# 0xEigenLabs/eigen-zkvm

Measured on AMD Instinct MI355X. Metric: Goldilocks NTT GElems/s + BN254 G1 MSM Mpts/s; starky prove ms at 2^24 rows, higher is better.
Workload: dtype u64 (Goldilocks, canonical)

## Files before the change

### eigen-zkvm_amd/csrc/ntt.hip

```cpp
#include "zk_internal.h"
#include "ntt_reg.hip.h"
#include <map>
#include <mutex>
#include <type_traits>
#include <vector>

namespace zk {

namespace {

constexpr int NTT_TILE = 4096;
constexpr int TW_LO_BITS = 12;
constexpr int TW_LO = 1 << TW_LO_BITS;

struct PassParams {
    const u64* in;
    u64* out;
    const u64* w256;
    const u64* tw_lo;
    const u64* tw_hi;
    const u64* tw_mid;
    u64 pre_scale;
    u32 dshift;
    const u64* sc_lo;
    const u64* sc_hi;
    u64 sc_cinv;
    u64 out_scale;
    u64 inner;
    u64 valid_in;
    u64 s_np;
    u32 np;
    u32 log_s;
    u32 has_tw;
};

__device__ __forceinline__ u64 tab2(const u64* __restrict__ lo, const u64* __restrict__ hi, u64 e) {
    return gl::mul_tw_nc(hi[e >> TW_LO_BITS], lo[e & (TW_LO - 1)]);
}

template <int LOGA, int LOGB, bool KMODE, bool INV>
__global__ __launch_bounds__(NTT_TILE / 16) void ntt_pass_kernel(const PassParams P) {
    constexpr int LOGR = LOGA + LOGB, R = 1 << LOGR, RA = 1 << LOGA, RB = 1 << LOGB;
    constexpr int C = NTT_TILE / R;
    constexpr int GA = 16 / RA, GB = 16 / RB;
    constexpr int TG = R / 16;
    constexpr int PAD = KMODE ? 512 / R : 0;
    constexpr int ROW = RB * C + PAD;
    static_assert(LOGR >= 4 && LOGR <= 8 && LOGA <= 4 && LOGB <= 4, "tile shape");
    __shared__ u64 lds[RA * ROW];
    __shared__ u64 sfac[RB * C];

    const int t = threadIdx.x;
    const u64 u0 = (u64)blockIdx.x * C;

    auto split = [&](u64 u, u64& p, u64& rem) {
        const u64 uc = u < P.inner ? u : 0;
        if (P.np == 1) { p = uc >> P.log_s; rem = uc & (((u64)1 << P.log_s) - 1); }
        else if ((P.inner >> 32) == 0) { const u32 p32 = (u32)uc / (u32)P.s_np; p = p32; rem = (u32)uc - p32 * (u32)P.s_np; }
        else
        { p = uc / P.s_np; rem = uc - p * P.s_np; }
    };
    auto row_of = [&](u64 rem) { return P.np == 1 ? rem : (P.inner >> 32) == 0 ? (u64)((u32)rem / P.np) : rem / P.np; };
    const bool small = ((P.inner * R) >> 29) == 0;
    int cB, tb;
    if (KMODE) { tb = t % TG; cB = t / TG; } else { cB = t % C; tb = t / C; }

    const bool split_f = (P.has_tw && !P.tw_mid) || P.sc_lo;
    u64 fa_hi[GB], fa_lo[GB], fs_hi[GA], fs_lo[GA], fa[GB];
#pragma unroll
    for (int g = 0; g < GB; ++g) fa_hi[g] = fa_lo[g] = fa[g] = 1;
#pragma unroll
    for (int m = 0; m < GA; ++m) fs_hi[m] = fs_lo[m] = 1;
    auto issue_factor_loads = [&]() {
        const u64* __restrict__ lo = P.sc_lo ? P.sc_lo : P.tw_lo;
        const u64* __restrict__ hi = P.sc_lo ? P.sc_hi : P.tw_hi;
        u64 p, rem;
        split(u0 + cB, p, rem);
        const u32 rq = P.sc_lo ? (u32)row_of(rem) : 0;
#pragma unroll
        for (int g = 0; g < GB; ++g) {
            const u32 ka = tb + g * TG;
            const u32 e = P.sc_lo ? (ka << P.log_s) + rq : ((u32)p * ka) << P.log_s;
            fa_hi[g] = hi[e >> TW_LO_BITS]; fa_lo[g] = lo[e & (TW_LO - 1)];
        }
#pragma unroll
        for (int m = 0; m < GA; ++m) {
            const int i = t + m * (NTT_TILE / 16);
            const u32 kb = i / C;
            split(u0 + i % C, p, rem);
            const u32 e = P.sc_lo ? (RA * kb) << P.log_s : ((u32)p * (RA * kb)) << P.log_s;
            fs_hi[m] = hi[e >> TW_LO_BITS]; fs_lo[m] = lo[e & (TW_LO - 1)];
        }
    };

    {
        const int c = t % C, ta = t / C;
        const u64 u = u0 + c;
        const bool live = u < P.inner;
        u64 x[GA][RA];
        const bool full = u0 + C <= P.inner && (u64)(R - 1) * P.inner + u0 + C <= P.valid_in;
        const u64* __restrict__ base = P.in + (u64)(ta * GA) * P.inner + (live ? u : 0);
        if (full) {
#pragma unroll
            for (int g = 0; g < GA; ++g)
#pragma unroll
                for (int ja = 0; ja < RA; ++ja) x[g][ja] = base[(u64)(ja * RB + g) * P.inner];
        } else {
#pragma unroll
            for (int g = 0; g < GA; ++g)
#pragma unroll
                for (int ja = 0; ja < RA; ++ja) {
                    const u64 off = (u64)(ja * RB + g) * P.inner;
                    const bool ok = live && (u64)(ta * GA) * P.inner + off + u < P.valid_in;
                    const u64 v = *(ok ? base + off : P.in);
                    x[g][ja] = ok ? v : 0;
                }
        }
        if (split_f) issue_factor_loads();
#pragma unroll
        for (int g = 0; g < GA; ++g) ntt_reg<LOGA, INV>(x[g]);
        if (LOGR <= 6 && C >= 64 && LOGB > 0 && P.pre_scale == 1) {
            static_for<0, TG>([&](auto TA) {
                constexpr int ta_c = decltype(TA)::value;
                if (ta == ta_c) {
                    static_for<0, GA>([&](auto GI) {
                        constexpr int g = decltype(GI)::value, jb = ta_c * GA + g;
                        static_for<0, RA>([&](auto KA) {
                            constexpr int ka = decltype(KA)::value;
                            constexpr int e0 = (39 * (64 / (R > 64 ? 64 : R)) * jb * ka) % 192, e = INV ? (192 - e0) % 192 : e0;
                            u64 v = x[g][bitrev_c(ka, LOGA)];
                            if constexpr (e >= 96) v = gl::neg(gl::mul_pow2<e - 96>(v));
                            else v = gl::mul_pow2<e>(v);
                            lds[ka * ROW + jb * C + c] = v;
                        });
                    });
                }
            });
        } else
        {
#pragma unroll
            for (int g = 0; g < GA; ++g) {
                const int jb = ta * GA + g;
#pragma unroll
                for (int ka = 0; ka < RA; ++ka) {
                    u64 v = x[g][bitrev_c(ka, LOGA)];
                    if (LOGB > 0 && ka > 0) v = gl::mul_tw(v, P.w256[(jb * ka) << (8 - LOGR)]);
                    else if (P.pre_scale != 1) v = gl::mul_tw(v, P.pre_scale);
                    lds[ka * ROW + jb * C + c] = v;
                }
            }
        }
    }
    if (split_f) {
#pragma unroll
        for (int m = 0; m < GA; ++m) {
            u64 sv = gl::mul_tw_nc(fs_hi[m], fs_lo[m]);
            if (P.sc_lo) sv = gl::mul_tw_nc(sv, P.sc_cinv);
            sfac[t + m * (NTT_TILE / 16)] = sv;
        }
#pragma unroll
        for (int g = 0; g < GB; ++g) fa[g] = gl::mul_tw_nc(fa_hi[g], fa_lo[g]);
    }
    __syncthreads();
    {
        const int c = cB;
        const u64 u = u0 + c;
        u64 y[GB][RB];
#pragma unroll
        for (int g = 0; g < GB; ++g) {
            const int ka = tb + g * TG;
#pragma unroll
            for (int jb = 0; jb < RB; ++jb) y[g][jb] = lds[ka * ROW + jb * C + c];
        }
        u64 p, rem;
        split(u, p, rem);
        u64 tw[GB][RB];
        if (P.tw_mid) {
            const u32 sh = P.log_s - P.dshift, istep = (((u32)p * RA) << sh) * 8;
#pragma unroll
            for (int g = 0; g < GB; ++g) {
                const u32 ka = tb + g * TG, i0 = (((u32)p * ka) << sh) * 8;
#pragma unroll
                for (int kb = 0; kb < RB; ++kb) tw[g][kb] = *(const u64*)((const char*)P.tw_mid + (u32)(i0 + kb * istep));
            }
        }
#pragma unroll
        for (int g = 0; g < GB; ++g) ntt_reg<LOGB, INV>(y[g]);
        if (u >= P.inner) return;

        auto finish = [&](auto small_c) {
            constexpr bool SMALL = decltype(small_c)::value;
            u64* __restrict__ outp = P.out + p * R * P.s_np + rem;
            const u64 kstride = P.s_np;
            const u32 b0 = ((u32)p * R * (u32)P.s_np + (u32)rem) * 8, bstep = RA * (u32)P.s_np * 8;
            auto put = [&](int g, int kb, u64 v) {
                const u32 ka = tb + g * TG;
                if constexpr (SMALL) *(u64*)((char*)P.out + (u32)(b0 + ka * (u32)P.s_np * 8 + kb * bstep)) = v;
                else outp[(u64)(RA * kb + ka) * kstride] = v;
            };
            if (P.tw_mid) {
#pragma unroll
                for (int g = 0; g < GB; ++g)
#pragma unroll
                    for (int kb = 0; kb < RB; ++kb) put(g, kb, gl::mul_tw(y[g][bitrev_c(kb, LOGB)], tw[g][kb]));
            } else if (split_f) {
#pragma unroll
                for (int g = 0; g < GB; ++g)
#pragma unroll
                    for (int kb = 0; kb < RB; ++kb) {
                        const u64 f = kb == 0 ? fa[g] : gl::mul_tw_nc(fa[g], sfac[kb * C + c]);
                        put(g, kb, gl::mul_tw(y[g][bitrev_c(kb, LOGB)], f));
                    }
            } else if (P.out_scale != 1) {
#pragma unroll
                for (int g = 0; g < GB; ++g)
#pragma unroll
                    for (int kb = 0; kb < RB; ++kb) put(g, kb, gl::mul_tw(y[g][bitrev_c(kb, LOGB)], P.out_scale));
            } else {
#pragma unroll
                for (int g = 0; g < GB; ++g)
#pragma unroll
                    for (int kb = 0; kb < RB; ++kb) put(g, kb, y[g][bitrev_c(kb, LOGB)]);
            }
        };
        if (small) finish(std::true_type{});
        else finish(std::false_type{});
    }
}

__global__ void ntt_small_kernel(const u64* in, u64* out, u32 np, u32 n_in, u32 n, u64 w, u64 g, u64 cst) {
    const u32 tid = blockIdx.x * blockDim.x + threadIdx.x;
    if (tid >= n * np) return;
    const u32 k = tid / np, c = tid % np;
    const u64 wk = gl::pow(w, k);
    u64 acc = 0, cur = 1;
    for (u32 i = 0; i < n_in; ++i) { acc = gl::add(acc, gl::mul(in[(u64)i * np + c], cur)); cur = gl::mul(cur, wk); }
    out[(u64)k * np + c] = gl::mul(acc, gl::mul(cst, gl::pow(g, k)));
}

struct Tables { DevConst w256, w256s, lo, hi, mid; u32 dshift = 0; };
struct ScaleTables { DevConst lo, hi; };

std::mutex g_mu;
auto& g_tables = *new std::map<std::pair<int, std::pair<u32, int>>, Tables>;
auto& g_scales = *new std::map<std::pair<int, std::pair<u32, u64>>, ScaleTables>;

void two_level(u64 base, u64 cst, u32 nbits, std::vector<u64>& lo, std::vector<u64>& hi) {
    lo.resize(TW_LO);
    u64 c = cst;
    for (int i = 0; i < TW_LO; ++i) { lo[i] = c; c = gl::hmul(c, base); }
    size_t nh = nbits > (u32)TW_LO_BITS ? (size_t)1 << (nbits - TW_LO_BITS) : 1;
    hi.resize(nh);
    u64 step = gl::hpow(base, TW_LO);
    c = 1;
    for (size_t i = 0; i < nh; ++i) { hi[i] = c; c = gl::hmul(c, step); }
}

const Tables& get_tables(u32 nbits, bool inverse) {
    int dev; ZK_HIP(hipGetDevice(&dev));
    std::lock_guard<std::mutex> lk(g_mu);
    auto key = std::make_pair(dev, std::make_pair(nbits, (int)inverse));
    auto it = g_tables.find(key);
    if (it != g_tables.end()) return it->second;
    u64 w = gl::hroot(nbits), w8 = gl::hroot(8);
    if (inverse) { w = gl::hinv(w); w8 = gl::hinv(w8); }
    std::vector<u64> t256(256), lo, hi;
    u64 c = 1;
    for (int i = 0; i < 256; ++i) { t256[i] = c; c = gl::hmul(c, w8); }
    two_level(w, 1, nbits, lo, hi);
    Tables T; T.w256 = DevConst(t256); T.lo = DevConst(lo); T.hi = DevConst(hi);
    if (inverse) {
        const u64 ninv = gl::hinv((1ull << nbits) % GL_P);
        std::vector<u64> t256s(256);
        for (int i = 0; i < 256; ++i) t256s[i] = gl::hmul(t256[i], ninv);
        T.w256s = DevConst(t256s);
    }
    {
        T.dshift = nbits > 16 ? nbits - 16 : 0;
        const size_t nm = (size_t)1 << (nbits - T.dshift);
        std::vector<u64> mid(nm);
        const u64 step = gl::hpow(w, 1ull << T.dshift);
        c = 1;
        for (size_t i = 0; i < nm; ++i) { mid[i] = c; c = gl::hmul(c, step); }
        T.mid = DevConst(mid);
    }
    return g_tables.emplace(key, std::move(T)).first->second;
}

const ScaleTables& get_scale(u32 nbits, u64 g, u64 cst) {
    int dev; ZK_HIP(hipGetDevice(&dev));
    std::lock_guard<std::mutex> lk(g_mu);
    auto key = std::make_pair(dev, std::make_pair(nbits, g));
    auto it = g_scales.find(key);
    if (it != g_scales.end()) return it->second;
    std::vector<u64> lo, hi;
    two_level(g, cst, nbits, lo, hi);
    ScaleTables S; S.lo = DevConst(lo); S.hi = DevConst(hi);
    return g_scales.emplace(key, std::move(S)).first->second;
}

template <int LOGA, int LOGB>
void launch_pass(const PassParams& P, bool kmode, bool inverse, hipStream_t st) {
    constexpr int C = NTT_TILE >> (LOGA + LOGB);
    const u64 blocks = (P.inner + C - 1) / C;
    ZK_REQUIRE(blocks < (1ull << 31), "ntt: grid too large");
    const dim3 g((u32)blocks), b(NTT_TILE / 16);
    const int variant = (kmode ? 2 : 0) | (inverse ? 1 : 0);
#define ZK_PASS(K, I) hipLaunchKernelGGL((ntt_pass_kernel<LOGA, LOGB, K, I>), g, b, 0, st, P)
    switch (variant) {
        case 0: ZK_PASS(false, false); break; case 1: ZK_PASS(false, true); break;
        case 2: ZK_PASS(true, false); break;  default: ZK_PASS(true, true); break;
    }
#undef ZK_PASS
    ZK_HIP(hipGetLastError());
}

void launch_pass_logr(int logr, const PassParams& P, bool kmode, bool inverse, hipStream_t st) {
    switch (logr) {
        case 4: launch_pass<2, 2>(P, kmode, inverse, st); break;
        case 5: launch_pass<3, 2>(P, kmode, inverse, st); break;
        case 6: launch_pass<3, 3>(P, kmode, inverse, st); break;
        case 7: launch_pass<4, 3>(P, kmode, inverse, st); break;
        case 8: launch_pass<4, 4>(P, kmode, inverse, st); break;
        default: throw Error("ntt: unsupported pass radix");
    }
}

std::vector<int> plan(u32 nbits) {
    std::vector<int> r;
    if (nbits < 4) return r;
    int np = (nbits + 7) / 8;
    int base = nbits / np, extra = nbits % np;
    for (int i = 0; i < np; ++i) r.push_back(base + (i < extra ? 1 : 0));
    return r;
}

struct Scale { bool on = false; u64 g = 1, cst = 1; };

void run_transform(const u64* in, u64* a, u64* b,
                   u32 n_pols, u32 nbits, u64 valid_rows, bool inverse, Scale sc, u64 out_scale, hipStream_t st) {
    const u64 n = 1ull << nbits;
    if (nbits < 4) {
        u64 w = gl::hroot(nbits);
        if (inverse) w = gl::hinv(w);
        u64 cst = sc.on ? sc.cst : out_scale;
        u64 g = sc.on ? sc.g : 1;
        u32 total = (u32)(n * n_pols);
        hipLaunchKernelGGL(ntt_small_kernel, dim3((total + 255) / 256), dim3(256), 0, st, in, a, n_pols,
                           (u32)valid_rows, (u32)n, w, g, cst);
        ZK_HIP(hipGetLastError());
        return;
    }
    const std::vector<int> radices = plan(nbits);
    const int np = (int)radices.size();
    const Tables& T = get_tables(nbits, inverse);
    const ScaleTables* S = sc.on ? &get_scale(nbits, sc.g, sc.cst) : nullptr;
    u32 log_s = 0;
    const u64* cur = in;
    for (int i = 0; i < np; ++i) {
        const int logr = radices[i];
        u64* dstbuf = ((np - 1 - i) % 2 == 0) ? a : b;
        const bool last = (i == np - 1);
        PassParams P{};
        P.in = cur; P.out = dstbuf;
        P.w256 = T.w256.u(); P.tw_lo = T.lo.u(); P.tw_hi = T.hi.u();
        P.sc_lo = (last && sc.on) ? S->lo.u() : nullptr;
        P.sc_hi = (last && sc.on) ? S->hi.u() : nullptr;
        P.sc_cinv = (last && sc.on) ? gl::hinv(sc.cst) : 1;
        P.out_scale = 1; P.pre_scale = 1;
        if (last && !sc.on && out_scale != 1) {
            ZK_REQUIRE(inverse && out_scale == gl::hinv(n % GL_P), "ntt: unsupported constant scaling");
            P.w256 = T.w256s.u(); P.pre_scale = out_scale;
        }
        P.inner = (n >> logr) * n_pols;
        P.valid_in = (i == 0) ? valid_rows * n_pols : n * n_pols;
        P.s_np = ((u64)1 << log_s) * n_pols;
        P.np = n_pols;
        P.log_s = log_s;
        P.has_tw = last ? 0 : 1;
        P.dshift = T.dshift;
        P.tw_mid = (!last && log_s >= T.dshift) ? T.mid.u() : nullptr;
        const bool kmode = P.s_np < 16;
        launch_pass_logr(logr, P, kmode, inverse, st);
        cur = dstbuf;
        log_s += logr;
    }
}

}

int ntt_num_passes(uint32_t nbits) { return nbits < 4 ? 1 : (int)plan(nbits).size(); }

const u64* ntt_w256_table(bool inverse) { return get_tables(8, inverse).w256.u(); }

void ntt_dev(const u64* d_src, u64* d_dst, u64* d_tmp, uint32_t n_pols, uint32_t nbits, bool inverse, hipStream_t st) {
    ZK_REQUIRE(nbits <= 32, "ntt: nbits > 32");
    if (n_pols == 0) return;
    ZK_REQUIRE(d_src != d_dst, "ntt: dst may not alias src");
    u64 out_scale = inverse ? gl::hinv((1ull << nbits) % GL_P) : 1;
    run_transform(d_src, d_dst, d_tmp, n_pols, nbits, 1ull << nbits, inverse, Scale{}, out_scale, st);
}

void lde_dev(const u64* d_src, u64* d_dst, u64* d_tmp, uint32_t n_pols, uint32_t nbits, uint32_t nbits_ext, hipStream_t st) {
    ZK_REQUIRE(nbits_ext <= 32 && nbits <= nbits_ext, "lde: need nbits <= nbits_ext <= 32");
    if (n_pols == 0) return;
    ZK_REQUIRE(d_src != d_dst, "lde: dst may not alias src");
    const u64 n = 1ull << nbits;
    Scale sc; sc.on = true; sc.g = 49; sc.cst = gl::hinv(n % GL_P);
    const int fwd_passes = ntt_num_passes(nbits_ext);
    u64* first_fwd_out = ((fwd_passes - 1) % 2 == 0) ? d_dst : d_tmp;
    u64* coef = (first_fwd_out == d_dst) ? d_tmp : d_dst;
    u64* other = (coef == d_dst) ? d_tmp : d_dst;
    run_transform(d_src, coef, other, n_pols, nbits, n, true, sc, 1, st);
    run_transform(coef, d_dst, d_tmp, n_pols, nbits_ext, n, false, Scale{}, 1, st);
}

}
```

Before: 80.96.

## Specialize NTT pass kernel on factor mode and index width at compile time

Adds template parameters for the factor mode (none, prescale, mid-table twiddles, split twiddle/scale) and the index-split mode. The host chooses a specialized instantiation for radix-128/256 passes when the data fits in 32-bit indexing. Specialized kernels do address math in u32, drop runtime branches and unused shared memory, and add sched_barriers so factor/twiddle loads are issued before the butterflies. This should cut registers and ALU work, at the cost of many more kernel instantiations and larger binaries.

```diff
diff --git a/eigen-zkvm_amd/csrc/ntt.hip b/eigen-zkvm_amd/csrc/ntt.hip
--- a/eigen-zkvm_amd/csrc/ntt.hip
+++ b/eigen-zkvm_amd/csrc/ntt.hip
@@ -38,7 +38,10 @@
     return gl::mul_tw_nc(hi[e >> TW_LO_BITS], lo[e & (TW_LO - 1)]);
 }
 
-template <int LOGA, int LOGB, bool KMODE, bool INV>
+constexpr int FM_ANY = 0, FM_NONE = 1, FM_PRESCALE = 2, FM_MID = 3, FM_SPLIT_TW = 4, FM_SPLIT_SC = 5;
+constexpr int LS_ANY = 0, LS_ONE_COL = 1, LS_DIV32 = 2;
+
+template <int LOGA, int LOGB, bool KMODE, bool INV, int FM, int LS>
 __global__ __launch_bounds__(NTT_TILE / 16) void ntt_pass_kernel(const PassParams P) {
     constexpr int LOGR = LOGA + LOGB, R = 1 << LOGR, RA = 1 << LOGA, RB = 1 << LOGB;
     constexpr int C = NTT_TILE / R;
@@ -46,41 +49,51 @@
     constexpr int TG = R / 16;
     constexpr int PAD = KMODE ? 512 / R : 0;
     constexpr int ROW = RB * C + PAD;
+    constexpr bool GEN = FM == FM_ANY;
     static_assert(LOGR >= 4 && LOGR <= 8 && LOGA <= 4 && LOGB <= 4, "tile shape");
+    static_assert((FM == FM_ANY) == (LS == LS_ANY), "the general form is general in both");
+    static_assert(INV || (FM != FM_PRESCALE && FM != FM_SPLIT_SC), "only inverse transforms scale");
+    using idx_t = std::conditional_t<GEN, u64, u32>;
     __shared__ u64 lds[RA * ROW];
-    __shared__ u64 sfac[RB * C];
+    __shared__ u64 sfac[GEN || FM == FM_SPLIT_TW || FM == FM_SPLIT_SC ? RB * C : 1];
 
     const int t = threadIdx.x;
-    const u64 u0 = (u64)blockIdx.x * C;
-
-    auto split = [&](u64 u, u64& p, u64& rem) {
-        const u64 uc = u < P.inner ? u : 0;
-        if (P.np == 1) { p = uc >> P.log_s; rem = uc & (((u64)1 << P.log_s) - 1); }
-        else if ((P.inner >> 32) == 0) { const u32 p32 = (u32)uc / (u32)P.s_np; p = p32; rem = (u32)uc - p32 * (u32)P.s_np; }
+    const idx_t u0 = (idx_t)blockIdx.x * C;
+    const idx_t inner = (idx_t)P.inner, s_np = (idx_t)P.s_np;
+    const bool one_col = GEN ? P.np == 1 : LS == LS_ONE_COL;
+    const bool div32 = GEN ? (P.inner >> 32) == 0 : true;
+    const bool f_sc = GEN ? P.sc_lo != nullptr : FM == FM_SPLIT_SC;
+    const bool f_mid = GEN ? P.tw_mid != nullptr : FM == FM_MID;
+    const bool f_pre = GEN ? P.pre_scale != 1 : FM == FM_PRESCALE;
+
+    auto split = [&](idx_t u, idx_t& p, idx_t& rem) {
+        const idx_t uc = u < inner ? u : 0;
+        if (one_col) { p = uc >> P.log_s; rem = uc & (((idx_t)1 << P.log_s) - 1); }
+        else if (div32) { const u32 p32 = (u32)uc / (u32)s_np; p = p32; rem = (u32)uc - p32 * (u32)s_np; }
         else
-        { p = uc / P.s_np; rem = uc - p * P.s_np; }
+        { p = uc / s_np; rem = uc - p * s_np; }
     };
-    auto row_of = [&](u64 rem) { return P.np == 1 ? rem : (P.inner >> 32) == 0 ? (u64)((u32)rem / P.np) : rem / P.np; };
-    const bool small = ((P.inner * R) >> 29) == 0;
+    auto row_of = [&](idx_t rem) { return one_col ? rem : div32 ? (idx_t)((u32)rem / P.np) : rem / P.np; };
+    const bool small = GEN ? ((P.inner * R) >> 29) == 0 : true;
     int cB, tb;
     if (KMODE) { tb = t % TG; cB = t / TG; } else { cB = t % C; tb = t / C; }
 
-    const bool split_f = (P.has_tw && !P.tw_mid) || P.sc_lo;
+    const bool split_f = GEN ? (P.has_tw && !P.tw_mid) || P.sc_lo : FM == FM_SPLIT_TW || FM == FM_SPLIT_SC;
     u64 fa_hi[GB], fa_lo[GB], fs_hi[GA], fs_lo[GA], fa[GB];
 #pragma unroll
     for (int g = 0; g < GB; ++g) fa_hi[g] = fa_lo[g] = fa[g] = 1;
 #pragma unroll
     for (int m = 0; m < GA; ++m) fs_hi[m] = fs_lo[m] = 1;
     auto issue_factor_loads = [&]() {
-        const u64* __restrict__ lo = P.sc_lo ? P.sc_lo : P.tw_lo;
-        const u64* __restrict__ hi = P.sc_lo ? P.sc_hi : P.tw_hi;
-        u64 p, rem;
+        const u64* __restrict__ lo = f_sc ? P.sc_lo : P.tw_lo;
+        const u64* __restrict__ hi = f_sc ? P.sc_hi : P.tw_hi;
+        idx_t p, rem;
         split(u0 + cB, p, rem);
-        const u32 rq = P.sc_lo ? (u32)row_of(rem) : 0;
+        const u32 rq = f_sc ? (u32)row_of(rem) : 0;
 #pragma unroll
         for (int g = 0; g < GB; ++g) {
             const u32 ka = tb + g * TG;
-            const u32 e = P.sc_lo ? (ka << P.log_s) + rq : ((u32)p * ka) << P.log_s;
+            const u32 e = f_sc ? (ka << P.log_s) + rq : ((u32)p * ka) << P.log_s;
             fa_hi[g] = hi[e >> TW_LO_BITS]; fa_lo[g] = lo[e & (TW_LO - 1)];
         }
 #pragma unroll
@@ -88,23 +101,32 @@
             const int i = t + m * (NTT_TILE / 16);
             const u32 kb = i / C;
             split(u0 + i % C, p, rem);
-            const u32 e = P.sc_lo ? (RA * kb) << P.log_s : ((u32)p * (RA * kb)) << P.log_s;
+            const u32 e = f_sc ? (RA * kb) << P.log_s : ((u32)p * (RA * kb)) << P.log_s;
             fs_hi[m] = hi[e >> TW_LO_BITS]; fs_lo[m] = lo[e & (TW_LO - 1)];
         }
     };
 
     {
         const int c = t % C, ta = t / C;
-        const u64 u = u0 + c;
-        const bool live = u < P.inner;
+        const idx_t u = u0 + c;
+        const bool live = u < inner;
         u64 x[GA][RA];
-        const bool full = u0 + C <= P.inner && (u64)(R - 1) * P.inner + u0 + C <= P.valid_in;
-        const u64* __restrict__ base = P.in + (u64)(ta * GA) * P.inner + (live ? u : 0);
+        const bool full = u0 + C <= inner && (u64)(R - 1) * P.inner + u0 + C <= P.valid_in;
+        const u64* __restrict__ base = P.in + (idx_t)(ta * GA) * inner + (live ? u : 0);
         if (full) {
-#pragma unroll
-            for (int g = 0; g < GA; ++g)
-#pragma unroll
-                for (int ja = 0; ja < RA; ++ja) x[g][ja] = base[(u64)(ja * RB + g) * P.inner];
+            if constexpr (GEN) {
+#pragma unroll
+                for (int g = 0; g < GA; ++g)
+#pragma unroll
+                    for (int ja = 0; ja < RA; ++ja) x[g][ja] = base[(u64)(ja * RB + g) * P.inner];
+            } else {
+                const u32 vo = ((u32)(ta * GA) * inner + u) * 8;
+#pragma unroll
+                for (int g = 0; g < GA; ++g)
+#pragma unroll
+                    for (int ja = 0; ja < RA; ++ja)
+                        x[g][ja] = *(const u64*)((const char*)P.in + (u64)((u32)(ja * RB + g) * inner) * 8 + vo);
+            }
         } else {
 #pragma unroll
             for (int g = 0; g < GA; ++g)
@@ -117,9 +139,11 @@
                 }
         }
         if (split_f) issue_factor_loads();
+        if constexpr (FM == FM_SPLIT_TW || FM == FM_SPLIT_SC) __builtin_amdgcn_sched_barrier(0);
 #pragma unroll
         for (int g = 0; g < GA; ++g) ntt_reg<LOGA, INV>(x[g]);
-        if (LOGR <= 6 && C >= 64 && LOGB > 0 && P.pre_scale == 1) {
+        u64* __restrict__ wbase = lds + (ta * GA) * C + c;
+        if (LOGR <= 6 && C >= 64 && LOGB > 0 && !f_pre) {
             static_for<0, TG>([&](auto TA) {
                 constexpr int ta_c = decltype(TA)::value;
                 if (ta == ta_c) {
@@ -131,7 +155,7 @@
                             u64 v = x[g][bitrev_c(ka, LOGA)];
                             if constexpr (e >= 96) v = gl::neg(gl::mul_pow2<e - 96>(v));
                             else v = gl::mul_pow2<e>(v);
-                            lds[ka * ROW + jb * C + c] = v;
+                            wbase[ka * ROW + g * C] = v;
                         });
                     });
                 }
@@ -145,8 +169,8 @@
                 for (int ka = 0; ka < RA; ++ka) {
                     u64 v = x[g][bitrev_c(ka, LOGA)];
                     if (LOGB > 0 && ka > 0) v = gl::mul_tw(v, P.w256[(jb * ka) << (8 - LOGR)]);
-                    else if (P.pre_scale != 1) v = gl::mul_tw(v, P.pre_scale);
-                    lds[ka * ROW + jb * C + c] = v;
+                    else if (f_pre) v = gl::mul_tw(v, P.pre_scale);
+                    wbase[ka * ROW + g * C] = v;
                 }
             }
         }
@@ -155,7 +179,7 @@
 #pragma unroll
         for (int m = 0; m < GA; ++m) {
             u64 sv = gl::mul_tw_nc(fs_hi[m], fs_lo[m]);
-            if (P.sc_lo) sv = gl::mul_tw_nc(sv, P.sc_cinv);
+            if (f_sc) sv = gl::mul_tw_nc(sv, P.sc_cinv);
             sfac[t + m * (NTT_TILE / 16)] = sv;
         }
 #pragma unroll
@@ -164,18 +188,17 @@
     __syncthreads();
     {
         const int c = cB;
-        const u64 u = u0 + c;
+        const idx_t u = u0 + c;
         u64 y[GB][RB];
-#pragma unroll
-        for (int g = 0; g < GB; ++g) {
-            const int ka = tb + g * TG;
-#pragma unroll
-            for (int jb = 0; jb < RB; ++jb) y[g][jb] = lds[ka * ROW + jb * C + c];
-        }
-        u64 p, rem;
+        const u64* __restrict__ rbase = lds + tb * ROW + c;
+#pragma unroll
+        for (int g = 0; g < GB; ++g)
+#pragma unroll
+            for (int jb = 0; jb < RB; ++jb) y[g][jb] = rbase[(g * TG) * ROW + jb * C];
+        idx_t p, rem;
         split(u, p, rem);
         u64 tw[GB][RB];
-        if (P.tw_mid) {
+        if (f_mid) {
             const u32 sh = P.log_s - P.dshift, istep = (((u32)p * RA) << sh) * 8;
 #pragma unroll
             for (int g = 0; g < GB; ++g) {
@@ -184,21 +207,23 @@
                 for (int kb = 0; kb < RB; ++kb) tw[g][kb] = *(const u64*)((const char*)P.tw_mid + (u32)(i0 + kb * istep));
             }
         }
+        if constexpr (FM == FM_MID) __builtin_amdgcn_sched_barrier(0);
 #pragma unroll
         for (int g = 0; g < GB; ++g) ntt_reg<LOGB, INV>(y[g]);
-        if (u >= P.inner) return;
+        if (u >= inner) return;
 
         auto finish = [&](auto small_c) {
             constexpr bool SMALL = decltype(small_c)::value;
-            u64* __restrict__ outp = P.out + p * R * P.s_np + rem;
+            u64* __restrict__ outp = P.out + p * R * s_np + rem;
             const u64 kstride = P.s_np;
             const u32 b0 = ((u32)p * R * (u32)P.s_np + (u32)rem) * 8, bstep = RA * (u32)P.s_np * 8;
             auto put = [&](int g, int kb, u64 v) {
                 const u32 ka = tb + g * TG;
-                if constexpr (SMALL) *(u64*)((char*)P.out + (u32)(b0 + ka * (u32)P.s_np * 8 + kb * bstep)) = v;
+                if constexpr (SMALL && !GEN) *(u64*)((char*)P.out + (u64)kb * bstep + (u32)(b0 + ka * (u32)P.s_np * 8)) = v;
+                else if constexpr (SMALL) *(u64*)((char*)P.out + (u32)(b0 + ka * (u32)P.s_np * 8 + kb * bstep)) = v;
                 else outp[(u64)(RA * kb + ka) * kstride] = v;
             };
-            if (P.tw_mid) {
+            if (f_mid) {
 #pragma unroll
                 for (int g = 0; g < GB; ++g)
 #pragma unroll
@@ -211,7 +236,7 @@
                         const u64 f = kb == 0 ? fa[g] : gl::mul_tw_nc(fa[g], sfac[kb * C + c]);
                         put(g, kb, gl::mul_tw(y[g][bitrev_c(kb, LOGB)], f));
                     }
-            } else if (P.out_scale != 1) {
+            } else if (GEN && P.out_scale != 1) {
 #pragma unroll
                 for (int g = 0; g < GB; ++g)
 #pragma unroll
@@ -224,7 +249,7 @@
             }
         };
         if (small) finish(std::true_type{});
-        else finish(std::false_type{});
+        else if constexpr (GEN) finish(std::false_type{});
     }
 }
 
@@ -299,19 +324,45 @@
     return g_scales.emplace(key, std::move(S)).first->second;
 }
 
+template <int LOGA, int LOGB, bool K, bool I, int FM, int LS>
+void launch_kernel(const PassParams& P, dim3 g, dim3 b, hipStream_t st) {
+    hipLaunchKernelGGL((ntt_pass_kernel<LOGA, LOGB, K, I, FM, LS>), g, b, 0, st, P);
+}
+
+template <int LOGA, int LOGB, bool K, bool I>
+void launch_mode(const PassParams& P, int fm, int ls, dim3 g, dim3 b, hipStream_t st) {
+#define ZK_PASS(FM) do { if (ls == LS_ONE_COL) launch_kernel<LOGA, LOGB, K, I, FM, LS_ONE_COL>(P, g, b, st); \
+                         else launch_kernel<LOGA, LOGB, K, I, FM, LS_DIV32>(P, g, b, st); return; } while (0)
+    if constexpr (LOGA + LOGB >= 7) if (ls != LS_ANY) {
+        if (fm == FM_MID) ZK_PASS(FM_MID);
+        if (fm == FM_SPLIT_TW) ZK_PASS(FM_SPLIT_TW);
+        if constexpr (I) {
+            if (fm == FM_PRESCALE) ZK_PASS(FM_PRESCALE);
+            if (fm == FM_SPLIT_SC) ZK_PASS(FM_SPLIT_SC);
+        } else {
+            if (fm == FM_NONE) ZK_PASS(FM_NONE);
+        }
+    }
+#undef ZK_PASS
+    launch_kernel<LOGA, LOGB, K, I, FM_ANY, LS_ANY>(P, g, b, st);
+}
+
 template <int LOGA, int LOGB>
 void launch_pass(const PassParams& P, bool kmode, bool inverse, hipStream_t st) {
-    constexpr int C = NTT_TILE >> (LOGA + LOGB);
+    constexpr int C = NTT_TILE >> (LOGA + LOGB), R = 1 << (LOGA + LOGB);
     const u64 blocks = (P.inner + C - 1) / C;
     ZK_REQUIRE(blocks < (1ull << 31), "ntt: grid too large");
     const dim3 g((u32)blocks), b(NTT_TILE / 16);
+    const int fm = P.sc_lo ? FM_SPLIT_SC : P.tw_mid ? FM_MID : P.has_tw ? FM_SPLIT_TW : P.pre_scale != 1 ? FM_PRESCALE
+                 : P.out_scale != 1 ? FM_ANY : FM_NONE;
+    const int ls = ((P.inner * R) >> 29) != 0 ? LS_ANY : P.np == 1 ? LS_ONE_COL : LS_DIV32;
     const int variant = (kmode ? 2 : 0) | (inverse ? 1 : 0);
-#define ZK_PASS(K, I) hipLaunchKernelGGL((ntt_pass_kernel<LOGA, LOGB, K, I>), g, b, 0, st, P)
     switch (variant) {
-        case 0: ZK_PASS(false, false); break; case 1: ZK_PASS(false, true); break;
-        case 2: ZK_PASS(true, false); break;  default: ZK_PASS(true, true); break;
-    }
-#undef ZK_PASS
+        case 0: launch_mode<LOGA, LOGB, false, false>(P, fm, ls, g, b, st); break;
+        case 1: launch_mode<LOGA, LOGB, false, true>(P, fm, ls, g, b, st); break;
+        case 2: launch_mode<LOGA, LOGB, true, false>(P, fm, ls, g, b, st); break;
+        default: launch_mode<LOGA, LOGB, true, true>(P, fm, ls, g, b, st); break;
+    }
     ZK_HIP(hipGetLastError());
 }
 
```

After: 82.22 (median of 6 runs). No clear change (+1.6%).
